# p-sawicki/entropy_coding

Hardware: AMD Instinct MI355X
Metric: Mbins/s encode+decode, intra QP32 synthetic bin buffers (higher is better)
Workload: dtype u32

## Files before the change

entropy_coding_amd/csrc/cabac_kernels_v4.hip:

```cpp
#include <cstdlib>
#include <type_traits>

#include "cabac_device.h"
#include "cabac_kernels.h"
#include "cabac_quad.h"

namespace cabac {


struct QuadEnc {
  uint64_t low;
  uint32_t range;
  int32_t pend;
  uint32_t buf;
  int32_t nbuf;
  uint32_t pos;
  uint8_t *dst;
  uint32_t cap;
};

__device__ __forceinline__ void quad_put_byte(QuadEnc &e, uint32_t byte, bool writer) {
  if (writer && e.pos < e.cap) e.dst[e.pos] = (uint8_t)byte;
  e.pos += 1;
}
// ... 84 lines not shown
}

__device__ __forceinline__ QuadEncInfo quad_unpack(uint32_t info) {
  QuadEncInfo f;
  f.k = info & 31u;
  f.c2 = (info >> 5) & 15u;
  f.lpsm = bit_mask<9>(info);
  f.ep = (info >> 10) & 1u;
  f.pem = bit_mask<11>(info);
  f.alm = bit_mask<12>(info);
  return f;
}

__device__ __forceinline__ uint32_t quad_enc_finish(QuadEnc &e, bool align_rbsp, bool writer, bool probe = false) {
  if (probe) return 8u * e.pos + 16u * (uint32_t)e.nbuf + (uint32_t)e.pend;
  const uint32_t total = (uint32_t)(9 + e.pend);
  if ((e.low >> total) & 1ull) {
    quad_put16(e, e.buf + 1u, writer);
    for (int32_t k = 1; k < e.nbuf; k++) quad_put16(e, 0x0000u, writer);
    e.low -= 1ull << total;
  } else {
    if (e.nbuf > 0) quad_put16(e, e.buf, writer);
    for (int32_t k = 1; k < e.nbuf; k++) quad_put16(e, 0xffffu, writer);
  }
  uint32_t nb = (uint32_t)(e.pend + 1);
  const uint32_t v = (uint32_t)(e.low >> 8);
  while (nb >= 8) {
    quad_put_byte(e, (v >> (nb - 8)) & 0xffu, writer);
    nb -= 8;
  }
  uint32_t held = nb ? ((v & ((1u << nb) - 1u)) << (8 - nb)) : 0u;
  if (align_rbsp) {
    held |= 1u << (7 - nb);
    quad_put_byte(e, held, writer);
    held = 0;
    nb = 0;
  }
  const uint32_t n_bits = e.pos * 8u + nb;
  if (nb) quad_put_byte(e, held, writer);
  return n_bits;
}

template <class... Sets>
__global__ __launch_bounds__(64) void encode_kernel_v4(uint32_t n_sub, const cabac_substream_desc *__restrict__ desc,
                                                       const uint16_t *__restrict__ records, uint8_t *__restrict__ bytes,
                                                       cabac_substream_result *__restrict__ results, Sets... sets) {
  constexpr bool kSets = sizeof...(Sets) != 0;
  constexpr bool kPieces = kQuadPieces<Sets...>;
  __shared__ uint32_t ctx[kQuadSubs * kQuadCtxStride];
  const uint32_t lane = threadIdx.x, row = lane >> 4, j = lane & 15u;
  const uint32_t sub = blockIdx.x * kQuadSubs + row;
  const QuadSetUse su = quad_set_use(sub, sub < n_sub, sets...);
  bool live = sub < n_sub && !su.bad;
  const cabac_substream_desc d = desc[live ? sub : 0];
  QuadPieceUse pu{};
  QuadSetUse su_out = su;
  if constexpr (kPieces) {
    pu = quad_piece_use<true>(sub, sub < n_sub, su.bad, d.byte_capacity, sets...);
    live = live && pu.code;
    if (pu.refuse) su_out.out = kNoSet;
  }
  const uint32_t n = live ? d.n_records : 0u;
  const uint16_t *rec = records + d.rec_offset;
  uint32_t *rctx = ctx + row * kQuadCtxStride;
  if constexpr (kSets) quad_ctx_load<true>(rctx, d.qp, d.init_id & 3u, j, 16u, su, sets...);
  else quad_ctx_init(rctx, d.qp, d.init_id & 3u, j);
  __syncthreads();

  QuadEnc e;
  e.low = 0;
  e.range = 510;
  e.pend = 0;
  e.buf = 0;
  e.nbuf = 0;
  e.pos = 0;
  if constexpr (kPieces) {
    e.low = pu.low;
    e.range = pu.range;
    e.pend = (int32_t)pu.pend;
    e.buf = pu.buf;
    e.nbuf = (int32_t)pu.nbuf;
    e.pos = pu.pos;
  }
  e.dst = bytes + d.byte_offset;
  e.cap = live ? d.byte_capacity : 0u;
  const bool writer = live && j == 0;
  uint32_t bad = 0;

  uint32_t next_rec = j < n ? rec[j] : 0;
  for (uint32_t base = 0; __ballot(base < n) != 0; base += 16) {
    const uint32_t r = next_rec;
    const uint32_t info = quad_phase_a(r, base + j < n, lane, row, rctx, bad);
    const QuadEncInfo f = quad_unpack(info);
    {
      const uint32_t nxt = base + 16u + j;
      next_rec = nxt < n ? rec[nxt] : 0;
    }
    if (__ballot(info >> 12) == 0) quad_enc_steps<false, false>(f, e, writer, QuadPost());
    else quad_enc_steps<true, false>(f, e, writer, QuadPost());
  }

  if constexpr (kPieces) {
    const CtxPieces &cp = quad_pack_first(sets...);
    const bool fin = (d.init_id & CABAC_SUB_FINISH) != 0;
    const uint32_t n_bits = live ? quad_enc_finish(e, (d.init_id & CABAC_SUB_ALIGN_RBSP) != 0, writer, !fin) : 0u;
    const uint64_t bad_mask = __ballot(bad != 0);
    const bool row_bad = ((bad_mask >> (row * 16u)) & 0xffffull) != 0;
    if (writer) {
      const uint32_t ends = fin ? e.pos : e.pos + 2u * (uint32_t)e.nbuf;
      cabac_substream_result res;
      res.n_bits = n_bits;
      res.flags = (ends > e.cap ? CABAC_RES_OVERFLOW : 0u) | (row_bad ? CABAC_RES_BAD_RECORD : 0u);
      results[sub] = res;
      if (fin) quad_piece_store(cp, sub, CABAC_CODER_CLOSED, res.flags, n_bits, e.pos, 0u, 0u, 0u, 0u);
      else quad_piece_store(cp, sub, CABAC_CODER_ENC, res.flags, n_bits, e.pos, (uint32_t)e.low, e.range | ((uint32_t)e.pend << 16), e.buf,
                            (uint32_t)e.nbuf);
    }
    quad_piece_pass(results, sub, sub < n_sub && j == 0, pu, cp);
    __syncthreads();
    quad_ctx_export(rctx, j, 16u, su_out, sets...);
    return;
  }
  const uint32_t n_bits = live ? quad_enc_finish(e, (d.init_id & CABAC_SUB_ALIGN_RBSP) != 0, writer, (d.init_id & CABAC_SUB_PROBE) != 0) : 0u;
  const uint64_t bad_mask = __ballot(bad != 0);
  const bool row_bad = ((bad_mask >> (row * 16u)) & 0xffffull) != 0;
  if (writer) {
    cabac_substream_result res;
    res.n_bits = n_bits;
    res.flags = (e.pos > e.cap ? CABAC_RES_OVERFLOW : 0u) | (row_bad ? CABAC_RES_BAD_RECORD : 0u);
    results[sub] = res;
  }
  if constexpr (kSets) {
    __syncthreads();
    quad_ctx_export(rctx, j, 16u, su, sets...);
    quad_bad_set_result(results, sub, j == 0, su);
  }
}

constexpr uint32_t kUnitSlots = 12;
constexpr uint32_t kUnitDump = 11;

template <int N>
__device__ __forceinline__ uint32_t row_shr(uint32_t v) {
  return (uint32_t)__builtin_amdgcn_update_dpp(0, (int)v, 0x110 + N, 0xf, 0xf, true);
}


struct QuadUnits {
  uint32_t m;
  uint64_t odd_rows;
  uint64_t store_lanes;
};

template <int kLanes = 16>
__device__ __forceinline__ QuadUnits quad_list_units(const QuadEnc &e, const uint32_t *plo, const uint32_t *phi,
                                                     const uint32_t *ppend, uint32_t row, uint32_t j, bool live,
                                                     uint32_t *list) {
  static_assert(kLanes == 16 || kLanes == 4, "a row or a quad per substream");
  const uint32_t c = (j & 3u) * kQuadSubs + row;
  const uint64_t low = ((uint64_t)phi[c] << 32) | plo[c];
  const uint32_t pend = ppend[c];
  const uint32_t nun = kLanes == 4 ? pend >> 4 : (pend >> 4) & neg_mask(j - 4u);
  const uint64_t v = low >> (9u + (pend & 15u));
  uint32_t incl = nun + (kLanes == 4 ? row_shr<1>(nun) & neg_mask(0u - j) : row_shr<1>(nun));
  incl += kLanes == 4 ? row_shr<2>(incl) & neg_mask(1u - j) : row_shr<2>(incl);
  const uint32_t idx = incl - nun;
  const uint32_t first = (uint32_t)(v >> (((nun - 1u) & 1u) << 4));
  const uint32_t second = (uint32_t)v & 0xffffu;
  const uint32_t has1 = neg_mask(0u - nun);
  const uint32_t has2 = neg_mask(1u - nun);
  list[sel(has1, idx, kUnitDump)] = first;
  list[sel(has2, idx + 1u, kUnitDump)] = second;
  QuadUnits u;
  u.m = group_bcast<kLanes, 3>(incl);
  const uint32_t room = e.cap - e.pos - 2u * u.m;
  uint32_t rowodd = neg_mask(0u - u.m) & (neg_mask(0u - ((uint32_t)e.nbuf ^ 1u)) | neg_mask(room));
  if (kLanes == 4) rowodd |= neg_mask(4u - u.m);
  u.odd_rows = __ballot(live && rowodd != 0);
  u.store_lanes = __ballot(live && j < u.m);
  return u;
}

__device__ __forceinline__ void quad_flush_list(QuadEnc &e, uint32_t m, const uint32_t *list, bool writer) {
  for (uint32_t k = 0; k < 8u && __ballot(k < m) != 0; k++) {
    if (k < m) quad_flush_lead(e, list[k], writer);
  }
}

__device__ __forceinline__ void quad_emit_units(QuadEnc &e, const QuadUnits &u, uint32_t j, const uint32_t *list,
                                                bool writer) {
  if (u.odd_rows != 0) return quad_flush_list(e, u.m, list, writer);
  const uint32_t act = neg_mask(j - u.m);
  const uint32_t jnz = neg_mask(0u - j);
  const uint32_t before = list[sel(act & jnz, j - 1u, kUnitDump)];
  const uint32_t mine = list[sel(act, j, kUnitDump)];
  const uint32_t last = list[sel(neg_mask(0u - u.m), u.m - 1u, kUnitDump)];
  const uint32_t x = (mine & 0x1ffffu) ^ 0xffffu;
  if (__ballot((act & neg_mask(x - 1u)) != 0) != 0) return quad_flush_list(e, u.m, list, writer);
  const uint32_t prev = sel(jnz, before & 0xffffu, e.buf);
  const uint32_t unit = prev + (mine >> 16);
  const uint32_t be = ((unit & 0xffu) << 8) | ((unit >> 8) & 0xffu);
  uint8_t *addr = e.dst + e.pos + 2u * j;
  uint64_t saved;
  asm volatile("s_mov_b64 %0, exec\n\ts_mov_b64 exec, %1\n\tglobal_store_short %2, %3, off\n\ts_mov_b64 exec, %0"
               : "=&s"(saved) : "s"(u.store_lanes), "v"(addr), "v"(be) : "memory");
  e.buf = sel(neg_mask(0u - u.m), last & 0xffffu, e.buf);
  e.pos += 2u * u.m;
}

#ifdef CABAC_V5_PROFILE
__device__ unsigned long long g_v5_prof[32];
#define V5_TICK(var) const unsigned long long var = __builtin_amdgcn_s_memtime()
#define V5_ADD(slot, t0, t1) \
  if (blockIdx.x == 0 && lane == 0) g_v5_prof[slot] += (t1) - (t0)
#define V5_HW_ID(w) \
  if (blockIdx.x == 0 && lane == 0) g_v5_prof[16 + (w)] = 0x100000000ull | (uint32_t)__builtin_amdgcn_s_getreg(4 | (31 << 11))
#else
#define V5_TICK(var)
#define V5_ADD(slot, t0, t1)
#define V5_HW_ID(w)
#endif
#ifndef CABAC_V5_STAMP_UNIT
#define CABAC_V5_STAMP_UNIT 0
#endif


struct QuadRngCap {
  uint32_t w[8];
};

template <int I, bool kAlign>
__device__ __forceinline__ void quad_rng_step(const QuadEncInfo &f, uint32_t &range, QuadRngCap &cap) {
  const uint32_t k = row_bcast<I>(f.k), c2 = row_bcast<I>(f.c2), lpsm = row_bcast<I>(f.lpsm);
  const uint32_t t = (__umul24((range >> 5) & 15u, k) + c2) >> 1;
  const uint32_t rm = range - t;
  const uint32_t x = sel(lpsm, t, rm);
  const uint32_t nb = (uint32_t)(__builtin_clz(x) - 23);
  range = x << nb;
  if (kAlign) range = sel(row_bcast<I>(f.alm), 256u, range);
  const uint32_t w = rm | (nb << 9);
  if (I & 1) cap.w[I >> 1] |= w << 16;
  else cap.w[I >> 1] = w;
}

struct QuadEncRow {
  uint32_t k[16], c2[16], lpsm[16];
};
template <int I, bool kAlign>
__device__ __forceinline__ void quad_rng_step_row(const QuadEncRow &u, const QuadEncInfo &f, uint32_t &range, QuadRngCap &cap) {
  const uint32_t t = (__umul24((range >> 5) & 15u, u.k[I]) + u.c2[I]) >> 1;
  const uint32_t rm = range - t;
  const uint32_t x = sel(u.lpsm[I], t, rm);
  const uint32_t nb = (uint32_t)(__builtin_clz(x) - 23);
  range = x << nb;
  if (kAlign) range = sel(row_bcast<I>(f.alm), 256u, range);
  const uint32_t w = rm | (nb << 9);
  if (I & 1) cap.w[I >> 1] |= w << 16;
  else cap.w[I >> 1] = w;
}
template <bool kAlign>
__device__ __forceinline__ void quad_rng_steps_row(const QuadEncRow &u, const QuadEncInfo &f, uint32_t &range, QuadRngCap &cap) {
#define QSTEP(I) quad_rng_step_row<I, kAlign>(u, f, range, cap)
  QSTEP(0); QSTEP(1); QSTEP(2); QSTEP(3); QSTEP(4); QSTEP(5); QSTEP(6); QSTEP(7);
  QSTEP(8); QSTEP(9); QSTEP(10); QSTEP(11); QSTEP(12); QSTEP(13); QSTEP(14); QSTEP(15);
#undef QSTEP
}

template <bool kAlign>
__device__ __forceinline__ void quad_rng_steps(const QuadEncInfo &f, uint32_t &range, QuadRngCap &cap) {
#define QSTEP(I) quad_rng_step<I, kAlign>(f, range, cap)
  QSTEP(0); QSTEP(1); QSTEP(2); QSTEP(3); QSTEP(4); QSTEP(5); QSTEP(6); QSTEP(7);
  QSTEP(8); QSTEP(9); QSTEP(10); QSTEP(11); QSTEP(12); QSTEP(13); QSTEP(14); QSTEP(15);
#undef QSTEP
}

__device__ __forceinline__ uint64_t shl64(uint32_t lo, uint32_t hi, uint32_t n) { return (((uint64_t)hi << 32) | lo) << n; }

__device__ __forceinline__ uint32_t quad_cap_mine(const QuadRngCap &cap, uint32_t j) {
  const uint32_t h = j >> 1;
  const uint32_t a0 = (h & 1u) ? cap.w[1] : cap.w[0], a1 = (h & 1u) ? cap.w[3] : cap.w[2], a2 = (h & 1u) ? cap.w[5] : cap.w[4],
                 a3 = (h & 1u) ? cap.w[7] : cap.w[6];
  const uint32_t b0 = (h & 2u) ? a1 : a0, b1 = (h & 2u) ? a3 : a2;
  const uint32_t pair = (h & 4u) ? b1 : b0;
  return ((j & 1u) ? pair >> 16 : pair) & 0xfffu;
}

__device__ __forceinline__ void quad_low_quads12(uint32_t w12, uint32_t info, uint32_t &v0, uint32_t &v1, uint32_t &s) {
  const uint32_t rm = w12 & 0x1ffu, nb = (w12 >> 9) & 7u;
  const uint32_t lpsm = bit_mask<9>(info), pem = bit_mask<11>(info), ep = (info >> 10) & 1u;
  const uint32_t term = ((rm & lpsm) << nb) | (rm & pem);
  s = nb + ep;
  uint64_t v = term;
  {
    const uint32_t p0 = row_shr<1>(term), ps = row_shr<1>(s);
    v = shl64(p0, 0u, s) + v;
    s += ps;
  }
  v0 = (uint32_t)v;
  {
    const uint32_t p0 = row_shr<2>(v0), ps = row_shr<2>(s);
    v = shl64(p0, 0u, s) + v;
    s += ps;
  }
  v0 = (uint32_t)v;
  v1 = (uint32_t)(v >> 32);
}

__device__ __forceinline__ void quad_low_quads(const QuadRngCap &cap, uint32_t info, uint32_t j, uint32_t &v0, uint32_t &v1,
                                               uint32_t &s) {
  quad_low_quads12(quad_cap_mine(cap, j), info, v0, v1, s);
}

__device__ __forceinline__ uint32_t quad_low_join(uint32_t v0, uint32_t v1, uint32_t s, uint32_t acc, uint32_t j, uint32_t (&out)[5]) {
  {
// ... 131 lines not shown
    if constexpr (kSets) {
      asm volatile("" ::: "memory");
      __builtin_amdgcn_wave_barrier();
      asm volatile("" ::: "memory");
      quad_ctx_export(rctx, j, 16u, su, sets...);
    }
    __syncthreads();
    __syncthreads();
  } else if (role == 1) {
    __builtin_amdgcn_s_setprio(CABAC_V6_PRIO_CHAIN);
    uint32_t range = 510;
    __syncthreads();
    for (uint32_t it = 0; it < n_iters; it++) {
      V5_TICK(t0);
#pragma unroll
      for (uint32_t h = 0; h < kSync; h++) {
        const uint32_t slot = (kSync * it + h) & (kRing - 1u);
        const uint32_t info = mail[slot][0][lane];
        QuadEncRow u;
#pragma unroll
        for (int q = 0; q < 4; q++) {
          lds_read4(&mail[slot][1][row * 16u], q, u.k);
          lds_read4(&mail[slot][2][row * 16u], q, u.c2);
          lds_read4(&mail[slot][3][row * 16u], q, u.lpsm);
        }
        QuadEncInfo f;
        f.alm = bit_mask<12>(info);
        QuadRngCap cap;
        if (__ballot(info >> 12) == 0) quad_rng_steps_row<false>(u, f, range, cap);
        else quad_rng_steps_row<true>(u, f, range, cap);
        if (kTreeInChain) {
          uint32_t q0, q1, qs;
          quad_low_quads(cap, info, j, q0, q1, qs);
          quad_post[unit][slot][0][lane] = q0;
          quad_post[unit][slot][1][lane] = q1;
          quad_post[unit][slot][2][lane] = qs;
        } else {
          quad_post[unit][slot][0][lane] = quad_cap_mine(cap, j);
          quad_post[unit][slot][1][lane] = info;
        }
      }
      V5_TICK(t1);
      __syncthreads();
      V5_TICK(t2);
      if (unit == 0) V5_ADD(4, t0, t1);
      if (unit == 0) V5_ADD(5, t1, t2);
    }
    __syncthreads();
    __syncthreads();
  } else if (role == 2) {
    __builtin_amdgcn_s_setprio(CABAC_V6_PRIO_LOW);
    uint32_t acc = 0, rem = 0;
    auto list_step = [&](uint32_t step) {
      const uint32_t slot = step & (kRing - 1u);
      uint32_t w[5];
      uint32_t q0 = quad_post[unit][slot][0][lane], q1 = quad_post[unit][slot][1][lane], qs;
      if (kTreeInChain) qs = quad_post[unit][slot][2][lane];
      else quad_low_quads12(q0, q1, q0, q1, qs);
      const uint32_t s_total = quad_low_join(q0, q1, qs, acc, j, w);
      const uint32_t pendn = rem + s_total, m = pendn >> 4;
      rem = pendn & 15u;
      const uint32_t base_off = 9u + rem;
      const uint32_t o = base_off + 16u * ((m - 1u - min(j, m - 1u)) & 7u);
      const uint32_t wi = o >> 5;
      const uint32_t lo = wi >= 2u ? (wi == 3u ? w[3] : w[2]) : (wi == 1u ? w[1] : w[0]);
      const uint32_t hi = wi >= 2u ? (wi == 3u ? w[4] : w[3]) : (wi == 1u ? w[2] : w[1]);
      const uint32_t lead = (uint32_t)((((uint64_t)hi << 32) | lo) >> (o & 31u)) & (j == 0u ? 0x1ffffu : 0xffffu);
      acc = m != 0u ? w[0] & ((1u << base_off) - 1u) : w[0];
      unit_list[unit][slot][row][j < m ? j : kUnitDump] = lead;
      if (j == 0u) unit_count[unit][slot][row] = m;
    };
    __syncthreads();
    for (uint32_t it = 0; it < n_iters; it++) {
      V5_TICK(t0);
      if (it != 0) {
#pragma unroll
        for (uint32_t h = 0; h < kSync; h++) list_step(kSync * (it - 1u) + h);
      }
      V5_TICK(t1);
      __syncthreads();
      V5_TICK(t2);
      if (unit == 0) V5_ADD(1, t0, t1);
      if (unit == 0) V5_ADD(7, t1, t2);
    }
    if (n_iters != 0) {
#pragma unroll
      for (uint32_t h = 0; h < kSync; h++) list_step(kSync * (n_iters - 1u) + h);
    }
    if (j == 0u) {
      fin_acc[unit][row] = acc;
      fin_rem[unit][row] = rem;
    }
    __syncthreads();
    __syncthreads();
  } else {
    __builtin_amdgcn_s_setprio(CABAC_V6_PRIO_EMIT);
    QuadEnc e;
    e.low = 0;
    e.range = 0;
    e.pend = 0;
    e.buf = 0;
    e.nbuf = 0;
    e.pos = 0;
    e.dst = bytes + d.byte_offset;
    e.cap = live ? d.byte_capacity : 0u;
    const bool writer = live && j == 0;
    auto emit_step = [&](uint32_t step) {
      const uint32_t slot = step & (kRing - 1u);
      const uint32_t *list = unit_list[unit][slot][row];
      QuadUnits u;
      u.m = unit_count[unit][slot][row];
      const uint32_t room = e.cap - e.pos - 2u * u.m;
      const uint32_t rowodd = neg_mask(0u - u.m) & (neg_mask(0u - ((uint32_t)e.nbuf ^ 1u)) | neg_mask(room));
      u.odd_rows = __ballot(rowodd != 0);
      u.store_lanes = __ballot(live && j < u.m);
      quad_emit_units(e, u, j, list, writer);
    };
    __syncthreads();
    for (uint32_t it = 0; it < n_iters; it++) {
      V5_TICK(t0);
      if (it >= 2u) {
#pragma unroll
        for (uint32_t h = 0; h < kSync; h++) emit_step(kSync * (it - 2u) + h);
      }
      V5_TICK(t1);
      __syncthreads();
      V5_TICK(t2);
      if (unit == 0) V5_ADD(0, t0, t1);
      if (unit == 0) V5_ADD(12, t1, t2);
    }
    if (n_iters >= 2u) {
#pragma unroll
      for (uint32_t h = 0; h < kSync; h++) emit_step(kSync * (n_iters - 2u) + h);
    }
    __syncthreads();
    if (n_iters != 0) {
#pragma unroll
      for (uint32_t h = 0; h < kSync; h++) emit_step(kSync * (n_iters - 1u) + h);
    }
    __syncthreads();
    e.low = fin_acc[unit][row];
    e.pend = (int32_t)fin_rem[unit][row];
    const uint32_t n_bits = live ? quad_enc_finish(e, (d.init_id & CABAC_SUB_ALIGN_RBSP) != 0, writer, (d.init_id & CABAC_SUB_PROBE) != 0) : 0u;
    if (writer) {
      cabac_substream_result res;
      res.n_bits = n_bits;
      res.flags = (e.pos > e.cap ? CABAC_RES_OVERFLOW : 0u) | (((bad_rows[unit] >> row) & 1u) ? CABAC_RES_BAD_RECORD : 0u);
      results[sub] = res;
    }
    if constexpr (kSets) quad_bad_set_result(results, sub, j == 0, su);
  }
}

constexpr uint32_t kV7Pad = 20;
enum : uint32_t { kV7K = 0, kV7C2, kV7Lpsm, kV7Lp9, kV7Ep, kV7Fields };

__device__ __forceinline__ uint32_t lane_rng_step(uint32_t k, uint32_t c2, uint32_t lpsm, uint32_t &range) {
  const uint32_t t = (__umul24((range >> 5) & 15u, k) + c2) >> 1;
  const uint32_t rm = range - t;
  const uint32_t x = sel(lpsm, t, rm);
  const uint32_t nb = (uint32_t)(__builtin_clz(x) - 23);
  range = x << nb;
  return (nb << 9) + rm;
}

template <int U, class... Sets>
__global__ __launch_bounds__(64 * (U + 3)) void encode_kernel_v7(uint32_t n_sub, const cabac_substream_desc *__restrict__ desc,
                                                                      const uint16_t *__restrict__ records,
                                                                      uint8_t *__restrict__ bytes,
                                                                      cabac_substream_result *__restrict__ results, Sets... sets) {
  constexpr bool kSets = sizeof...(Sets) != 0;
  constexpr bool kPieces = kQuadPieces<Sets...>;
  constexpr uint32_t S = U * kQuadSubs;
  __shared__ uint32_t ctx_all[S * kQuadCtxStride];
  __shared__ __attribute__((aligned(16))) uint32_t fld[4][kV7Fields][S * kV7Pad];
  __shared__ __attribute__((aligned(16))) uint32_t wpost[2][(S + 1) * kV7Pad];
  __shared__ uint32_t post_lo[U][2][4 * kQuadSubs], post_hi[U][2][4 * kQuadSubs], post_pend[U][2][4 * kQuadSubs];
  __shared__ uint32_t fin_lo[S], fin_hi[S], fin_pend[S];
  __shared__ uint32_t fin_range[S];
  __shared__ uint32_t unit_list[U][kQuadSubs][kUnitSlots];
  constexpr bool kKinds = U == 4;
  constexpr uint32_t kMatch = kKinds ? kMatchWordsCtx : kMatchWords;
  __shared__ uint32_t match_all[U][kMatch];
  __shared__ __attribute__((aligned(16))) uint4 kind_tab[kKinds ? kKindRows : 1];
  __shared__ uint2 rate_tab[kKinds ? 1 : 512];
  __shared__ uint32_t bad_rows[U];
  __shared__ uint32_t wg_max_n;
  const uint32_t wave = threadIdx.x >> 6, lane = threadIdx.x & 63u;
  V5_HW_ID(wave);
  if constexpr (kKinds) quad_kind_tab_init(kind_tab, threadIdx.x, blockDim.x);
  else quad_rate_tab_init(rate_tab, threadIdx.x, blockDim.x);
  constexpr bool kLdsMatch = true;
  for (uint32_t k = threadIdx.x; k < U * kMatch; k += blockDim.x) (&match_all[0][0])[k] = 0u;
  constexpr uint32_t kChainWave = U == 4 ? 3u : 1u, kLowWave = U == 4 ? 5u : 2u, kOutWave = U == 4 ? 6u : 3u;
  const bool is_chain = wave == kChainWave, is_low = wave == kLowWave, is_out = wave == kOutWave;
  const bool is_ctx = !is_chain && !is_low && !is_out;
  uint32_t row, j, unit, local;
  bool in_range = true;
  if (is_ctx) {
    row = lane >> 4;
    j = lane & 15u;
    unit = min(wave, U - 1u);
    local = unit * kQuadSubs + row;
  } else if (is_chain) {
    row = lane >> 4;
    j = lane & 15u;
    unit = 0;
    in_range = lane < S;
    local = min(lane, S - 1u);
  } else {
    const uint32_t g = lane >> 2;
    in_range = g < S;
    local = min(g, S - 1u);
    unit = local >> 2;
    row = local & 3u;
    j = lane & 3u;
  }
  const uint32_t sub = blockIdx.x * S + local;
  const QuadSetUse su = quad_set_use(sub, sub < n_sub, sets...);
  bool in_batch = sub < n_sub && !su.bad;
  const cabac_substream_desc d = desc[in_batch ? sub : 0];
  QuadPieceUse piece{};
  QuadSetUse su_out = su;
  if constexpr (kPieces) {
    piece = quad_piece_use<true>(sub, sub < n_sub, su.bad, d.byte_capacity, sets...);
    in_batch = in_batch && piece.code;
    if (piece.refuse) su_out.out = kNoSet;
  }
  const bool live = in_batch && in_range;
  const uint32_t n = in_batch ? d.n_records : 0u;

  if (threadIdx.x == 0) wg_max_n = 0;
  __syncthreads();
  atomicMax(&wg_max_n, n);
  __syncthreads();
  const uint32_t max_n = wg_max_n;
  const uint32_t n_steps = (max_n + 15u) >> 4;

  if (is_ctx) {
    const uint16_t *rec = records + d.rec_offset;
    uint32_t *rctx = ctx_all + local * kQuadCtxStride;
    if constexpr (kSets) quad_ctx_load<true>(rctx, d.qp, d.init_id & 3u, j, 16u, su, sets...);
    else quad_ctx_init(rctx, d.qp, d.init_id & 3u, j);
    uint32_t bad = 0;
    const uint16_t *rec_safe = n != 0 ? rec : reinterpret_cast<const uint16_t *>(desc);
    const uint32_t last_rec = n != 0 ? n - 1u : 0u;
    const uint32_t at = local * kV7Pad + j;
    auto post = [&](uint32_t slot, const QuadFields &f) {
      fld[slot][kV7K][at] = f.k;
      fld[slot][kV7C2][at] = f.c2;
      fld[slot][kV7Lpsm][at] = f.lpsm;
      fld[slot][kV7Lp9][at] = f.lp9;
      fld[slot][kV7Ep][at] = f.ep;
    };
    const uint32_t cur_rec = rec_safe[min(j, last_rec)];
    uint32_t next_rec = rec_safe[min(16u + j, last_rec)];
    uint32_t ahead1 = rec_safe[min(32u + j, last_rec)], ahead2 = rec_safe[min(48u + j, last_rec)], ahead3 = rec_safe[min(64u + j, last_rec)];
    post(0, quad_phase_fields<kLdsMatch, kKinds>(cur_rec, j < n, lane, row, rctx, bad, match_all[unit], rate_tab, kind_tab));
    __syncthreads();
    for (uint32_t k = 0; k < n_steps; k++) {
      const uint32_t base = 16u * k;
      const uint32_t r = next_rec;
      next_rec = ahead1;
      ahead1 = ahead2;
      ahead2 = ahead3;
      ahead3 = rec_safe[min(base + 80u + j, last_rec)];
      V5_TICK(t0);
      post((k + 1u) & 3u, quad_phase_fields<kLdsMatch, kKinds>(r, base + 16u + j < n, lane, row, rctx, bad, match_all[unit], rate_tab, kind_tab));
      V5_TICK(t1);
      __syncthreads();
      V5_TICK(t2);
      if (unit == CABAC_V5_STAMP_UNIT) V5_ADD(0, t0, t1);
      if (unit == CABAC_V5_STAMP_UNIT) V5_ADD(1, t1, t2);
    }
    const uint64_t bad_mask = __ballot(bad != 0);
    if (lane == 0) {
      uint32_t rows = 0;
      for (uint32_t q = 0; q < 4; q++) rows |= ((bad_mask >> (16u * q)) & 0xffffull) ? (1u << q) : 0u;
      bad_rows[unit] = rows;
    }
    if constexpr (kSets) {
      asm volatile("" ::: "memory");
      __builtin_amdgcn_wave_barrier();
      asm volatile("" ::: "memory");
      quad_ctx_export(rctx, j, 16u, su_out, sets...);
    }
    __syncthreads();
    __syncthreads();
  } else if (is_chain) {
    __builtin_amdgcn_s_setprio(3);
    uint32_t range = 510;
    if constexpr (kPieces) range = piece.range;
    __syncthreads();
    for (uint32_t k = 0; k < n_steps; k++) {
      V5_TICK(t0);
      const uint32_t slot = k & 3u;
      uint32_t kk[16], c2[16], lm[16], w[16];
#pragma unroll
      for (int q = 0; q < 4; q++) {
        lds_read4(&fld[slot][kV7K][local * kV7Pad], q, kk);
        lds_read4(&fld[slot][kV7C2][local * kV7Pad], q, c2);
        lds_read4(&fld[slot][kV7Lpsm][local * kV7Pad], q, lm);
      }
#pragma unroll
      for (int i = 0; i < 16; i++) w[i] = lane_rng_step(kk[i], c2[i], lm[i], range);
      uint4 *dst = reinterpret_cast<uint4 *>(&wpost[k & 1u][min(lane, S) * kV7Pad]);
#pragma unroll
      for (int i = 0; i < 4; i++) dst[i] = make_uint4(w[4 * i], w[4 * i + 1], w[4 * i + 2], w[4 * i + 3]);
      V5_TICK(t1);
      __syncthreads();
      V5_TICK(t2);
      V5_ADD(2, t0, t1);
      V5_ADD(3, t1, t2);
    }
    if constexpr (kPieces) fin_range[local] = range;
    __syncthreads();
    __syncthreads();
  } else if (is_low) {
    uint64_t low = 0;
    uint32_t pend = 0;
    if constexpr (kPieces) {
      low = piece.low;
      pend = piece.pend;
    }
    const uint32_t pu = local >> 2, pr = local & 3u, q = j;
    auto quad_from_left = [](uint32_t v) {
      return (uint32_t)__builtin_amdgcn_update_dpp(0, (int)v, 0x90, 0xf, 0xf, true);
    };
    auto low_step = [&](uint32_t k) {
      const uint32_t slot = k & 3u;
      const uint4 w4 = reinterpret_cast<const uint4 *>(&wpost[k & 1u][local * kV7Pad])[q];
      const uint4 l4 = reinterpret_cast<const uint4 *>(&fld[slot][kV7Lp9][local * kV7Pad])[q];
      const uint4 e4 = reinterpret_cast<const uint4 *>(&fld[slot][kV7Ep][local * kV7Pad])[q];
      const uint32_t w[4] = {w4.x, w4.y, w4.z, w4.w}, lp9[4] = {l4.x, l4.y, l4.z, l4.w}, ep[4] = {e4.x, e4.y, e4.z, e4.w};
      uint32_t term[4], sh[4];
#pragma unroll
      for (int i = 0; i < 4; i++) {
        const uint32_t nb = w[i] >> 9;
        term[i] = (w[i] & lp9[i]) << nb;
        sh[i] = nb + ep[i];
      }
      const uint32_t p01 = (term[0] << sh[1]) + term[1];
      const uint64_t P = ((((uint64_t)p01 << sh[2]) + term[2]) << sh[3]) + term[3];
      const uint32_t Ssum = sh[0] + sh[1] + sh[2] + sh[3];
      uint64_t cut = 0, posted = 0;
      uint32_t cut_pend = 0, posted_pend = 0;
#pragma unroll
      for (int r = 0; r < 4; r++) {
        uint64_t in = low;
        uint32_t in_pend = pend;
        if (r != 0) {
          const uint32_t lo = quad_from_left((uint32_t)cut), hi = quad_from_left((uint32_t)(cut >> 32)), pp = quad_from_left(cut_pend);
          in = q == 0 ? low : ((uint64_t)hi << 32) | lo;
          in_pend = q == 0 ? pend : pp;
        }
        posted = (in << Ssum) + P;
        posted_pend = in_pend + Ssum;
        const uint32_t keep = posted_pend & 15u;
        const uint32_t width = posted_pend >= 16u ? 9u + keep : 63u;
        cut = posted & ~(~0ull << width);
        cut_pend = keep;
      }
      const uint32_t c = q * kQuadSubs + pr;
      post_lo[pu][k & 1u][c] = (uint32_t)posted;
      post_hi[pu][k & 1u][c] = (uint32_t)(posted >> 32);
      post_pend[pu][k & 1u][c] = posted_pend;
      low = ((uint64_t)group_bcast<4, 3>((uint32_t)(cut >> 32)) << 32) | group_bcast<4, 3>((uint32_t)cut);
      pend = group_bcast<4, 3>(cut_pend);
    };
    __syncthreads();
    for (uint32_t k = 0; k < n_steps; k++) {
      V5_TICK(t0);
      if (k != 0) low_step(k - 1u);
      V5_TICK(t1);
      __syncthreads();
      V5_TICK(t2);
      V5_ADD(4, t0, t1);
      V5_ADD(5, t1, t2);
    }
    if (n_steps != 0) low_step(n_steps - 1u);
    fin_lo[local] = (uint32_t)low;
    fin_hi[local] = (uint32_t)(low >> 32);
    fin_pend[local] = pend;
    __syncthreads();
    __syncthreads();
  } else {
    QuadEnc e;
    e.low = 0;
    e.range = 0;
    e.pend = 0;
    e.buf = 0;
    e.nbuf = 0;
    e.pos = 0;
    if constexpr (kPieces) {
      e.buf = piece.buf;
      e.nbuf = (int32_t)piece.nbuf;
      e.pos = piece.pos;
    }
    e.dst = bytes + d.byte_offset;
    e.cap = live ? d.byte_capacity : 0u;
    const bool writer = live && j == 0;
    uint32_t *list = unit_list[unit][row];
    QuadUnits units;
    units.m = 0;
    units.odd_rows = 0;
    units.store_lanes = 0;
    bool listed = false;
    auto list_step = [&](uint32_t k) {
      units = quad_list_units<4>(e, post_lo[unit][k & 1u], post_hi[unit][k & 1u], post_pend[unit][k & 1u], row, j, live, list);
    };
    __builtin_amdgcn_s_waitcnt(0x0f70);
    __syncthreads();
    for (uint32_t k = 0; k < n_steps; k++) {
      V5_TICK(t0);
      if (listed) quad_emit_units(e, units, j, list, writer);
      listed = k >= 2u;
      if (listed) list_step(k - 2u);
      V5_TICK(t1);
      __syncthreads();
      V5_TICK(t2);
      V5_ADD(6, t0, t1);
      V5_ADD(7, t1, t2);
    }
    if (listed) quad_emit_units(e, units, j, list, writer);
    if (n_steps >= 2u) {
      list_step(n_steps - 2u);
      quad_emit_units(e, units, j, list, writer);
    }
    __syncthreads();
    if (n_steps != 0) {
      list_step(n_steps - 1u);
      quad_emit_units(e, units, j, list, writer);
    }
    e.low = ((uint64_t)fin_hi[local] << 32) | fin_lo[local];
    e.pend = (int32_t)fin_pend[local];
    if constexpr (kPieces) {
      __syncthreads();
      const CtxPieces &cp = quad_pack_first(sets...);
      const bool fin = (d.init_id & CABAC_SUB_FINISH) != 0;
      const uint32_t n_bits = live ? quad_enc_finish(e, (d.init_id & CABAC_SUB_ALIGN_RBSP) != 0, writer, !fin) : 0u;
      if (writer) {
        const uint32_t ends = fin ? e.pos : e.pos + 2u * (uint32_t)e.nbuf;
        cabac_substream_result res;
        res.n_bits = n_bits;
        res.flags = (ends > e.cap ? CABAC_RES_OVERFLOW : 0u) | (((bad_rows[unit] >> row) & 1u) ? CABAC_RES_BAD_RECORD : 0u);
        results[sub] = res;
        if (fin) quad_piece_store(cp, sub, CABAC_CODER_CLOSED, res.flags, n_bits, e.pos, 0u, 0u, 0u, 0u);
        else quad_piece_store(cp, sub, CABAC_CODER_ENC, res.flags, n_bits, e.pos, (uint32_t)e.low, fin_range[local] | ((uint32_t)e.pend << 16),
                              e.buf, (uint32_t)e.nbuf);
      }
      quad_piece_pass(results, sub, sub < n_sub && in_range && j == 0, piece, cp);
      return;
    }
    const uint32_t n_bits = live ? quad_enc_finish(e, (d.init_id & CABAC_SUB_ALIGN_RBSP) != 0, writer, (d.init_id & CABAC_SUB_PROBE) != 0) : 0u;
    if (writer) {
      cabac_substream_result res;
      res.n_bits = n_bits;
      res.flags = (e.pos > e.cap ? CABAC_RES_OVERFLOW : 0u) | (((bad_rows[unit] >> row) & 1u) ? CABAC_RES_BAD_RECORD : 0u);
      results[sub] = res;
    }
    if constexpr (kSets) quad_bad_set_result(results, sub, in_range && j == 0, su);
    __syncthreads();
  }
}


struct QuadDec {
  uint32_t hi, lo;
  uint32_t used;
  uint32_t range;
  uint32_t npos;
  uint32_t q_hi, q_lo;
  uint32_t *ring;
  uint32_t filled;
  uint32_t pf_data, pf_off, pf_mask;
  const uint8_t *src;
  uint32_t cap;
  const uint8_t *src_safe;
  uint32_t last_dword;
};

struct QuadDecInfo {
  uint32_t c2;
  uint32_t ep;
  uint32_t srmul;
  uint32_t ctxm;
  uint32_t ntrm;
  uint32_t alm;
  uint32_t key;
};

__device__ __forceinline__ void quad_dec_topup(QuadDec &w) {
  const uint64_t q = (((uint64_t)w.q_hi << 32) | w.q_lo) << (~w.npos & 31u);
  const uint32_t next32 = (uint32_t)(q >> 32);
  const uint32_t want = w.used;
  uint32_t add;
  asm("v_bfe_u32 %0, %1, %2, %3" : "=v"(add) : "v"(next32), "v"(32u - want), "v"(want));
  w.lo |= add;
  w.npos -= want;
  w.used = 0;
  const uint32_t *p = w.ring + ((w.npos >> 5) & 63u);
  w.q_lo = p[0];
  w.q_hi = p[1];
}

template <int L = 16>
__device__ __forceinline__ void quad_dec_stage_load(QuadDec &w, uint32_t j) {
  constexpr uint32_t kLanes = L > 16 ? 16u : (uint32_t)L;
  const uint32_t wanted = neg_mask(w.filled - (~w.npos >> 3) - 128u);
  w.pf_mask = L > 16 ? wanted & neg_mask(j - kLanes) : wanted;
  w.pf_off = w.filled + 4u * (j & (kLanes - 1u));
  w.pf_data = *reinterpret_cast<const uint32_t *>(w.src_safe + min(w.pf_off, w.last_dword));
  w.filled += (4u * kLanes) & wanted;
}
__device__ __forceinline__ void quad_dec_stage_store(QuadDec &w) {
  const uint32_t v = __builtin_bswap32(w.pf_data) & neg_mask(w.pf_off - w.cap);
  const uint32_t at = (w.pf_off >> 2) & 63u;
  w.ring[sel(w.pf_mask, 64u - at, 65u)] = v;
  w.ring[sel(w.pf_mask & neg_mask(at - 1u), 0u, 65u)] = v;
}

constexpr uint32_t kRingStride = 66;

template <int L = 16>
struct QuadDecRow {
  static constexpr int kN = L > 16 ? 16 : L;
  uint32_t c2[kN], ctxm[kN], srmul[kN], ep[kN], key[kN];
  __device__ __forceinline__ void fetch(const uint32_t *fields, uint32_t at) {
    auto one = [&](uint32_t which, uint32_t (&dst)[kN]) {
      const uint4 *p = reinterpret_cast<const uint4 *>(fields + which * 64u + at);
#pragma unroll
      for (int q = 0; q < kN / 4; q++) {
        const uint4 v = p[q];
        dst[4 * q] = v.x;
        dst[4 * q + 1] = v.y;
        dst[4 * q + 2] = v.z;
        dst[4 * q + 3] = v.w;
      }
    };
    one(0, c2);
    one(1, ctxm);
    one(2, key);
    one(3, srmul);
    one(4, ep);
  }
};

#ifndef CABAC_PAIR_PICK
#define CABAC_PAIR_PICK 4
#endif
constexpr int kPairPick = CABAC_PAIR_PICK;
constexpr int kPairEvery = kPairPick > 0 ? kPairPick : 1;
struct QuadDecPair {
  uint32_t d;
  uint32_t d0, d1;
  uint32_t p1;
};
__device__ __forceinline__ uint32_t quad_dec_derived(uint32_t st) {
  const uint32_t sum = (st & 0xffffu) + (st >> 16);
  const uint32_t sx = (uint32_t)((int32_t)(sum << 16) >> 31);
  return (((sum >> 10) ^ sx) & 31u) | (sx & 0x80000000u);
}

template <int I, bool kSpecial, int L = 16, bool kPairs = false>
__device__ __forceinline__ void quad_dec_step(const QuadDecInfo &f, const QuadDecRow<L> &u, uint32_t r0_v, uint32_t a_v, uint32_t &st_v,
                                              uint32_t (&bits)[2], QuadDec &w, QuadDecPair *pr = nullptr) {
  constexpr int J = I % QuadDecRow<L>::kN;
  if constexpr (kPairs) {
    static_assert(L == 16 && !kSpecial, "the pairs variant is the quad decoder's, without special records");
    const uint32_t dw = group_bcast<L, I>(pr->d);
// ... 834 lines not shown
```

Before: 90510.

## Deepen v7 encode pipeline: context waves run two steps ahead, chain prefetches fields

Context waves now compute and post phase fields two steps ahead into the four-slot ring instead of one, with the record prefetch window shifted to match. The chain wave is unrolled by two, so it reads the next step's k/c2/lpsm from LDS before running the current step's range recurrence. This hides LDS latency behind the serial range chain. The emit wave now loads its post words at the top of each step, before emitting units, so those LDS reads overlap the emit work. The cost is more register pressure on the chain wave, and correctness now relies on the four ring slots being enough for the wider lookahead.

```diff
diff --git a/entropy_coding_amd/csrc/cabac_kernels_v4.hip b/entropy_coding_amd/csrc/cabac_kernels_v4.hip
--- a/entropy_coding_amd/csrc/cabac_kernels_v4.hip
+++ b/entropy_coding_amd/csrc/cabac_kernels_v4.hip
@@ -260,14 +260,25 @@
   uint64_t store_lanes;
 };
 
+struct QuadPostWords {
+  uint32_t lo, hi, pend;
+};
+__device__ __forceinline__ QuadPostWords quad_post_load(const uint32_t *plo, const uint32_t *phi, const uint32_t *ppend,
+                                                        uint32_t row, uint32_t j) {
+  const uint32_t c = (j & 3u) * kQuadSubs + row;
+  QuadPostWords p;
+  p.lo = plo[c];
+  p.hi = phi[c];
+  p.pend = ppend[c];
+  return p;
+}
+
 template <int kLanes = 16>
-__device__ __forceinline__ QuadUnits quad_list_units(const QuadEnc &e, const uint32_t *plo, const uint32_t *phi,
-                                                     const uint32_t *ppend, uint32_t row, uint32_t j, bool live,
+__device__ __forceinline__ QuadUnits quad_list_units(const QuadEnc &e, const QuadPostWords &p, uint32_t row, uint32_t j, bool live,
                                                      uint32_t *list) {
   static_assert(kLanes == 16 || kLanes == 4, "a row or a quad per substream");
-  const uint32_t c = (j & 3u) * kQuadSubs + row;
-  const uint64_t low = ((uint64_t)phi[c] << 32) | plo[c];
-  const uint32_t pend = ppend[c];
+  const uint64_t low = ((uint64_t)p.hi << 32) | p.lo;
+  const uint32_t pend = p.pend;
   const uint32_t nun = kLanes == 4 ? pend >> 4 : (pend >> 4) & neg_mask(j - 4u);
   const uint64_t v = low >> (9u + (pend & 15u));
   uint32_t incl = nun + (kLanes == 4 ? row_shr<1>(nun) & neg_mask(0u - j) : row_shr<1>(nun));
@@ -705,6 +716,10 @@
   }
 }
 
+constexpr uint32_t kV7Ring = 4;
+static_assert(kV7Ring == 4, "a slot each for: the context waves' write two steps ahead, the chain wave's read-ahead, the step "
+                            "whose lp9 / ep planes wait for the low wave, and the step the low wave reads — no fewer, and the "
+                            "slot arithmetic (& 3) is written for four");
 constexpr uint32_t kV7Pad = 20;
 enum : uint32_t { kV7K = 0, kV7C2, kV7Lpsm, kV7Lp9, kV7Ep, kV7Fields };
 
@@ -726,7 +741,7 @@
   constexpr bool kPieces = kQuadPieces<Sets...>;
   constexpr uint32_t S = U * kQuadSubs;
   __shared__ uint32_t ctx_all[S * kQuadCtxStride];
-  __shared__ __attribute__((aligned(16))) uint32_t fld[4][kV7Fields][S * kV7Pad];
+  __shared__ __attribute__((aligned(16))) uint32_t fld[kV7Ring][kV7Fields][S * kV7Pad];
   __shared__ __attribute__((aligned(16))) uint32_t wpost[2][(S + 1) * kV7Pad];
   __shared__ uint32_t post_lo[U][2][4 * kQuadSubs], post_hi[U][2][4 * kQuadSubs], post_pend[U][2][4 * kQuadSubs];
   __shared__ uint32_t fin_lo[S], fin_hi[S], fin_pend[S];
@@ -807,9 +822,11 @@
       fld[slot][kV7Ep][at] = f.ep;
     };
     const uint32_t cur_rec = rec_safe[min(j, last_rec)];
-    uint32_t next_rec = rec_safe[min(16u + j, last_rec)];
-    uint32_t ahead1 = rec_safe[min(32u + j, last_rec)], ahead2 = rec_safe[min(48u + j, last_rec)], ahead3 = rec_safe[min(64u + j, last_rec)];
+    const uint32_t second_rec = rec_safe[min(16u + j, last_rec)];
+    uint32_t next_rec = rec_safe[min(32u + j, last_rec)];
+    uint32_t ahead1 = rec_safe[min(48u + j, last_rec)], ahead2 = rec_safe[min(64u + j, last_rec)], ahead3 = rec_safe[min(80u + j, last_rec)];
     post(0, quad_phase_fields<kLdsMatch, kKinds>(cur_rec, j < n, lane, row, rctx, bad, match_all[unit], rate_tab, kind_tab));
+    post(1, quad_phase_fields<kLdsMatch, kKinds>(second_rec, 16u + j < n, lane, row, rctx, bad, match_all[unit], rate_tab, kind_tab));
     __syncthreads();
     for (uint32_t k = 0; k < n_steps; k++) {
       const uint32_t base = 16u * k;
@@ -817,9 +834,9 @@
       next_rec = ahead1;
       ahead1 = ahead2;
       ahead2 = ahead3;
-      ahead3 = rec_safe[min(base + 80u + j, last_rec)];
+      ahead3 = rec_safe[min(base + 96u + j, last_rec)];
       V5_TICK(t0);
-      post((k + 1u) & 3u, quad_phase_fields<kLdsMatch, kKinds>(r, base + 16u + j < n, lane, row, rctx, bad, match_all[unit], rate_tab, kind_tab));
+      post((k + 2u) & (kV7Ring - 1u), quad_phase_fields<kLdsMatch, kKinds>(r, base + 32u + j < n, lane, row, rctx, bad, match_all[unit], rate_tab, kind_tab));
       V5_TICK(t1);
       __syncthreads();
       V5_TICK(t2);
@@ -844,22 +861,53 @@
     __builtin_amdgcn_s_setprio(3);
     uint32_t range = 510;
     if constexpr (kPieces) range = piece.range;
-    __syncthreads();
-    for (uint32_t k = 0; k < n_steps; k++) {
-      V5_TICK(t0);
-      const uint32_t slot = k & 3u;
-      uint32_t kk[16], c2[16], lm[16], w[16];
+    struct V7ChainFields {
+      uint32_t kk[16], c2[16], lm[16];
+    };
+    auto read_fields = [&](uint32_t step, V7ChainFields &f) {
+      const uint32_t slot = step & (kV7Ring - 1u);
 #pragma unroll
       for (int q = 0; q < 4; q++) {
-        lds_read4(&fld[slot][kV7K][local * kV7Pad], q, kk);
-        lds_read4(&fld[slot][kV7C2][local * kV7Pad], q, c2);
-        lds_read4(&fld[slot][kV7Lpsm][local * kV7Pad], q, lm);
+        lds_read4(&fld[slot][kV7K][local * kV7Pad], q, f.kk);
+        lds_read4(&fld[slot][kV7C2][local * kV7Pad], q, f.c2);
+        lds_read4(&fld[slot][kV7Lpsm][local * kV7Pad], q, f.lm);
       }
+    };
+    auto chain_step = [&](uint32_t k, const V7ChainFields &f) {
+      uint32_t w[16];
 #pragma unroll
-      for (int i = 0; i < 16; i++) w[i] = lane_rng_step(kk[i], c2[i], lm[i], range);
+      for (int i = 0; i < 16; i++) w[i] = lane_rng_step(f.kk[i], f.c2[i], f.lm[i], range);
       uint4 *dst = reinterpret_cast<uint4 *>(&wpost[k & 1u][min(lane, S) * kV7Pad]);
 #pragma unroll
       for (int i = 0; i < 4; i++) dst[i] = make_uint4(w[4 * i], w[4 * i + 1], w[4 * i + 2], w[4 * i + 3]);
+    };
+    auto hold_range = [&]() { asm volatile("" : "+v"(range)); };
+    V7ChainFields fa, fb;
+    __syncthreads();
+    if (n_steps != 0) read_fields(0u, fa);
+    uint32_t k = 0;
+    for (; k + 2u <= n_steps; k += 2u) {
+      V5_TICK(t0);
+      read_fields(k + 1u, fb);
+      chain_step(k, fa);
+      V5_TICK(t1);
+      __syncthreads();
+      hold_range();
+      V5_TICK(t2);
+      read_fields(k + 2u, fa);
+      chain_step(k + 1u, fb);
+      V5_TICK(t3);
+      __syncthreads();
+      hold_range();
+      V5_TICK(t4);
+      V5_ADD(2, t0, t1);
+      V5_ADD(3, t1, t2);
+      V5_ADD(2, t2, t3);
+      V5_ADD(3, t3, t4);
+    }
+    if (k < n_steps) {
+      V5_TICK(t0);
+      chain_step(k, fa);
       V5_TICK(t1);
       __syncthreads();
       V5_TICK(t2);
@@ -959,16 +1007,16 @@
     units.odd_rows = 0;
     units.store_lanes = 0;
     bool listed = false;
-    auto list_step = [&](uint32_t k) {
-      units = quad_list_units<4>(e, post_lo[unit][k & 1u], post_hi[unit][k & 1u], post_pend[unit][k & 1u], row, j, live, list);
-    };
+    auto load_step = [&](uint32_t k) { return quad_post_load(post_lo[unit][k & 1u], post_hi[unit][k & 1u], post_pend[unit][k & 1u], row, j); };
+    auto list_step = [&](uint32_t k) { units = quad_list_units<4>(e, load_step(k), row, j, live, list); };
     __builtin_amdgcn_s_waitcnt(0x0f70);
     __syncthreads();
     for (uint32_t k = 0; k < n_steps; k++) {
       V5_TICK(t0);
+      const QuadPostWords posts = load_step(k);
       if (listed) quad_emit_units(e, units, j, list, writer);
       listed = k >= 2u;
-      if (listed) list_step(k - 2u);
+      if (listed) units = quad_list_units<4>(e, posts, row, j, live, list);
       V5_TICK(t1);
       __syncthreads();
       V5_TICK(t2);
```

Measured after the change: 90200. Within noise of the previous version (-0.3%).
